# dohlee/rosettafold-pytorch

Measured on AMD Instinct MI355X. Metric: residues/sec forward (L=256, N=128), higher is better.
Workload: dtype bf16; 1 GPU; BASELINE.json configs[1]: bsz=4/GPU, n_seq=128, L=256, d_msa=384, d_pair=288, 8+5 blocks, 4 encoder layers, random-init weights; global_batch=4, parallelism=batch-sharded x1 (replicated weights), launch=one hipGraph replay per step (validation + input copy outside the graph)

## Files before the change

rosettafold-pytorch_amd/csrc/favor.hip:

```cpp
#include <type_traits>

#include "common.h"

#define FV_DH 64
#define FV_M 266
#define FV_MT 17
#define FV_MPAD 288
#define FV_CTX_LD 592
#define FV_DT 5
#define FV_DROWS 80

struct FavorAttnP {
  const h16_t* qkv;
  const h16_t* pc;
  h16_t* out;
  int64_t x_b, x_o, x_s;
  int64_t x_h;
  int64_t o_b, o_o, o_s;
  int q_off, k_off, v_off;
  int n_o, n_h, nitems;
  int nchunks;
  int dbg;
  float eps;
  float ctx_scale;
  int seq_len;
};

#ifdef RF_H16_IS_F16
#define FV_CS(x) ((x) * p.ctx_scale)
#else
#define FV_CS(x) (x)
#endif

typedef __attribute__((ext_vector_type(4))) short s16x4;

__device__ __forceinline__ int swz_off(int row, int chunk) { return row * 128 + ((chunk ^ (row & 7)) << 4); }

template <bool TAIL = false>
__device__ __forceinline__ void fv_load_tile(char* smem, int lds_off, const h16_t* g, int64_t stride, int nrows,
                                             int wave, int lane, int nvalid = 0) {
  const int ninstr = nrows * 8 / 64;
  for (int it = wave; it < ninstr; it += 4) {
    const int slot = it * 64 + lane;
    const int row = slot >> 3;
    const int clog = (slot & 7) ^ (row & 7);
    const int srow = TAIL ? (row < nvalid ? row : nvalid - 1) : row;
    rf_glds16(g + (int64_t)srow * stride + clog * 8, smem + lds_off + it * 1024);
  }
}

__device__ __forceinline__ float rbf(float x) { return h2f(f2h(x)); }

__device__ __forceinline__ float fv_mfma_done(float acc_reg) {
  asm volatile("s_nop 7\n\ts_nop 3" : "+v"(acc_reg));
  return acc_reg;
}

union Frag {
  h16x8 v;
  unsigned u[4];
  uint2 h[2];
};

template <int LS, bool SOFTMAX, bool TAIL>
__global__ __launch_bounds__(256, 1) void favor_attention_kernel(const FavorAttnP p) {
  constexpr int ST = LS / 64;
  constexpr int NSB = LS / 32;
  constexpr int PC_OFF = 0;
  constexpr int K_OFF = FV_MPAD * 128;
  constexpr int V_OFF = K_OFF + LS * 128;
  constexpr int CTX_OFF = V_OFF + LS * 128;
  constexpr int DIAG_OFF = CTX_OFF + FV_DROWS * FV_CTX_LD;
  constexpr int RED_OFF = DIAG_OFF + LS * 4;
  extern __shared__ __attribute__((aligned(16))) char smem[];
  const int tid = threadIdx.x, lane = tid & 63;
  const int wave = __builtin_amdgcn_readfirstlane(tid >> 6) & 3;
  const int fr = lane & 15, fq = lane >> 4;
  const int nm = wave == 0 ? 5 : 4;
  const int m0t = wave == 0 ? 0 : 5 + 4 * (wave - 1);
  const f32x4 epsv = {p.eps, p.eps, p.eps, p.eps};
  Frag ones;
#pragma unroll
  for (int k = 0; k < 4; ++k) ones.u[k] = fr == 0 ? RF_H16_ONE2 : 0u;

  fv_load_tile(smem, PC_OFF, p.pc, FV_DH, FV_MPAD, wave, lane);
  for (int i = tid; i < FV_DROWS * FV_CTX_LD / 4; i += 256) ((unsigned*)(smem + CTX_OFF))[i] = 0u;

  auto item_base = [&](int item, int64_t& xb, int64_t& ob) {
    const int h = item % p.n_h;
    const int t = item / p.n_h;
    const int o = t % p.n_o, b = t / p.n_o;
    xb = (int64_t)b * p.x_b + (int64_t)o * p.x_o + (int64_t)h * p.x_h;
    ob = (int64_t)b * p.o_b + (int64_t)o * p.o_o + h * FV_DH;
  };

  const int nch = p.nchunks;
  const int nv = TAIL ? p.seq_len : 0;
  int item = blockIdx.x;
  if (item < p.nitems) {
    int64_t xb, ob;
    item_base(item, xb, ob);
    fv_load_tile<TAIL>(smem, K_OFF, p.qkv + xb + p.k_off, p.x_s, LS, wave, lane, nv);
    fv_load_tile<TAIL>(smem, V_OFF, p.qkv + xb + p.v_off, p.x_s, LS, wave, lane, nv);
  }
  bool first = true;
  for (; item < p.nitems; item += gridDim.x) {
    int64_t xb, ob;
    item_base(item, xb, ob);
    if (first || TAIL)
      asm volatile("s_waitcnt vmcnt(0)" ::: "memory");
    else
      asm volatile("s_waitcnt vmcnt(%0)" ::"n"(ST * 4) : "memory");
    first = false;
    __syncthreads();
    h16x8 qf[ST][2];
    auto load_q = [&](int chunk) {
#pragma unroll
      for (int t = 0; t < ST; ++t) {
        int s = chunk * LS + (wave * ST + t) * 16 + fr;
        if (TAIL) s = s < nv ? s : nv - 1;
        const h16_t* qrow = p.qkv + xb + p.q_off + (int64_t)s * p.x_s;
#pragma unroll
        for (int kk = 0; kk < 2; ++kk) qf[t][kk] = *(const h16x8*)(qrow + (kk * 4 + fq) * 8);
      }
    };
    load_q(0);

    float gmax = 0.f;
    if constexpr (SOFTMAX) {
      for (int s = tid; s < LS; s += 256) {
        float a = 0.f;
#pragma unroll
        for (int c = 0; c < 8; ++c) {
          const h16x8 x = *(const h16x8*)(smem + K_OFF + s * 128 + c * 16);
#pragma unroll
          for (int e = 0; e < 8; ++e) {
            const float f = h2f((h16_t)x[e]);
            a = fmaf(f, f, a);
          }
        }
        ((float*)(smem + DIAG_OFF))[s] = a * (0.0625f * 1.4426950408889634f);
      }
    }

    h16x8 pf[5][2];
#pragma unroll
    for (int j = 0; j < 5; ++j)
#pragma unroll
      for (int kk = 0; kk < 2; ++kk)
        if (j < nm) pf[j][kk] = *(const h16x8*)(smem + PC_OFF + swz_off((m0t + j) * 16 + fr, kk * 4 + fq));

    if constexpr (SOFTMAX) {
      float mx = -INFINITY;
      const int nsb0 = TAIL ? (nv + 31) >> 5 : NSB;
      for (int u = 0; u < nsb0; ++u) {
        h16x8 kf[2][2];
#pragma unroll
        for (int t = 0; t < 2; ++t)
#pragma unroll
          for (int kk = 0; kk < 2; ++kk)
            kf[t][kk] = *(const h16x8*)(smem + K_OFF + swz_off((2 * u + t) * 16 + fr, kk * 4 + fq));
#pragma unroll
        for (int j = 0; j < 5; ++j) {
          if (j < nm) {
            const bool valid = (m0t + j) * 16 + fr < FV_M;
#pragma unroll
            for (int t = 0; t < 2; ++t) {
              f32x4 a = {0.f, 0.f, 0.f, 0.f};
              a = rf_mfma16(kf[t][0], pf[j][0], a, 0, 0, 0);
              a = rf_mfma16(kf[t][1], pf[j][1], a, 0, 0, 0);
              if (valid) mx = fmaxf(mx, fmaxf(fmaxf(a[0], a[1]), fmaxf(a[2], a[3])));
            }
          }
        }
      }
      mx = wave_max(mx);
      if (lane == 0) ((float*)(smem + RED_OFF))[wave] = mx;
      __syncthreads();
      const float* red = (const float*)(smem + RED_OFF);
      gmax = fmaxf(fmaxf(red[0], red[1]), fmaxf(red[2], red[3]));
    }

    f32x4 ctx[5][FV_DT];
#pragma unroll
    for (int j = 0; j < 5; ++j)
#pragma unroll
      for (int i = 0; i < FV_DT; ++i) ctx[j][i] = (f32x4){0.f, 0.f, 0.f, 0.f};
    for (int ck = 0; ck < nch; ++ck) {
    const int rem = TAIL ? nv - ck * LS : LS;
    if (ck > 0) {
      __syncthreads();
      fv_load_tile<TAIL>(smem, K_OFF, p.qkv + xb + p.k_off + (int64_t)ck * LS * p.x_s, p.x_s, LS, wave, lane, rem);
      fv_load_tile<TAIL>(smem, V_OFF, p.qkv + xb + p.v_off + (int64_t)ck * LS * p.x_s, p.x_s, LS, wave, lane, rem);
      asm volatile("s_waitcnt vmcnt(0)" ::: "memory");
      __syncthreads();
    }
    const int nsb = TAIL ? (rem < LS ? (rem + 31) >> 5 : NSB) : NSB;
    for (int u = 0; u < nsb; ++u) {
      h16x8 kf[2][2];
#pragma unroll
      for (int t = 0; t < 2; ++t)
#pragma unroll
        for (int kk = 0; kk < 2; ++kk)
          kf[t][kk] = *(const h16x8*)(smem + K_OFF + swz_off((2 * u + t) * 16 + fr, kk * 4 + fq));
      Frag vf[4];
      {
        const int p4 = fr & 3;
#pragma unroll
        for (int i = 0; i < 4; ++i) {
#pragma unroll
          for (int half = 0; half < 2; ++half) {
            const int row = u * 32 + half * 16 + 4 * fq + (fr >> 2);
            const int off = V_OFF + swz_off(row, i * 2 + (p4 >> 1)) + (p4 & 1) * 8;
            const s16x4 r = __builtin_amdgcn_ds_read_tr16_b64_v4i16((__attribute__((address_space(3))) s16x4*)(smem + off));
            vf[i].h[half] = __builtin_bit_cast(uint2, r);
          }
        }
      }
      f32x4 init[2] = {epsv, epsv};
      if constexpr (SOFTMAX) {
#pragma unroll
        for (int t = 0; t < 2; ++t) {
          const float4 d4 = *(const float4*)(smem + DIAG_OFF + ((2 * u + t) * 16 + 4 * fq) * 4);
          init[t] = (f32x4){-(d4.x + gmax), -(d4.y + gmax), -(d4.z + gmax), -(d4.w + gmax)};
        }
      }
#pragma unroll
      for (int j = 0; j < 5; ++j) {
        if (j < nm) {
          f32x4 a[2];
#pragma unroll
          for (int t = 0; t < 2; ++t) {
            a[t] = rf_mfma16(kf[t][0], pf[j][0], init[t], 0, 0, 0);
            a[t] = rf_mfma16(kf[t][1], pf[j][1], a[t], 0, 0, 0);
          }
          float f[2][4];
#pragma unroll
          for (int t = 0; t < 2; ++t)
#pragma unroll
            for (int r = 0; r < 4; ++r) {
              if constexpr (SOFTMAX)
                f[t][r] = __builtin_amdgcn_exp2f(a[t][r]) + p.eps;
              else
                f[t][r] = fmaxf(a[t][r], p.eps);
            }
          if ((m0t + j) == FV_MT - 1 && fr >= FV_M - 16 * (FV_MT - 1)) {
#pragma unroll
            for (int t = 0; t < 2; ++t)
#pragma unroll
              for (int r = 0; r < 4; ++r) f[t][r] = 0.f;
          }
          if constexpr (TAIL) {
            if ((u + 1) * 32 > rem) {
#pragma unroll
              for (int t = 0; t < 2; ++t)
#pragma unroll
                for (int r = 0; r < 4; ++r) f[t][r] = (2 * u + t) * 16 + 4 * fq + r < rem ? f[t][r] : 0.f;
            }
          }
          Frag kfr;
          kfr.u[0] = rf_pack2_h16(f[0][0], f[0][1]);
          kfr.u[1] = rf_pack2_h16(f[0][2], f[0][3]);
          kfr.u[2] = rf_pack2_h16(f[1][0], f[1][1]);
          kfr.u[3] = rf_pack2_h16(f[1][2], f[1][3]);
#pragma unroll
          for (int i = 0; i < 4; ++i)
            ctx[j][i] = rf_mfma16(kfr.v, vf[i].v, ctx[j][i], 0, 0, 0);
          ctx[j][4] = rf_mfma16(kfr.v, ones.v, ctx[j][4], 0, 0, 0);
        }
      }
    }
    }
#pragma unroll
    for (int j = 0; j < 5; ++j) {
      if (j < nm) {
#pragma unroll
        for (int i = 0; i < FV_DT; ++i) {
          uint2 w;
          w.x = rf_pack2_h16(FV_CS(ctx[j][i][0]), FV_CS(ctx[j][i][1]));
          w.y = rf_pack2_h16(FV_CS(ctx[j][i][2]), FV_CS(ctx[j][i][3]));
          *(uint2*)(smem + CTX_OFF + (i * 16 + fr) * FV_CTX_LD + ((m0t + j) * 16 + 4 * fq) * 2) = w;
        }
      }
    }
    __syncthreads();

    asm volatile("s_waitcnt vmcnt(0)" ::: "memory");
    {
      const int nxt = item + gridDim.x;
      if (nxt < p.nitems) {
        int64_t xb2, ob2;
        item_base(nxt, xb2, ob2);
        fv_load_tile<TAIL>(smem, K_OFF, p.qkv + xb2 + p.k_off, p.x_s, LS, wave, lane, nv);
        fv_load_tile<TAIL>(smem, V_OFF, p.qkv + xb2 + p.v_off, p.x_s, LS, wave, lane, nv);
      }
    }

    f32x4 qinit[ST];
#pragma unroll
    for (int t = 0; t < ST; ++t) qinit[t] = epsv;
    if constexpr (SOFTMAX) {
      float dq[ST], rmax[ST];
#pragma unroll
      for (int t = 0; t < ST; ++t) {
        float a = 0.f;
#pragma unroll
        for (int kk = 0; kk < 2; ++kk)
#pragma unroll
          for (int e = 0; e < 8; ++e) {
            const float f = h2f((h16_t)qf[t][kk][e]);
            a = fmaf(f, f, a);
          }
        a += __shfl_xor(a, 16, 64);
        a += __shfl_xor(a, 32, 64);
        dq[t] = a * (0.0625f * 1.4426950408889634f);
        rmax[t] = -INFINITY;
      }
      for (int j = 0; j < FV_MT; ++j) {
        h16x8 pfr[2];
#pragma unroll
        for (int kk = 0; kk < 2; ++kk) pfr[kk] = *(const h16x8*)(smem + PC_OFF + swz_off(j * 16 + fr, kk * 4 + fq));
#pragma unroll
        for (int t = 0; t < ST; ++t) {
          f32x4 a = {0.f, 0.f, 0.f, 0.f};
          a = rf_mfma16(pfr[0], qf[t][0], a, 0, 0, 0);
          a = rf_mfma16(pfr[1], qf[t][1], a, 0, 0, 0);
#pragma unroll
          for (int r = 0; r < 4; ++r)
            if (j * 16 + 4 * fq + r < FV_M) rmax[t] = fmaxf(rmax[t], a[r]);
        }
      }
#pragma unroll
      for (int t = 0; t < ST; ++t) {
        rmax[t] = fmaxf(rmax[t], __shfl_xor(rmax[t], 16, 64));
        rmax[t] = fmaxf(rmax[t], __shfl_xor(rmax[t], 32, 64));
        const float off = -(dq[t] + rmax[t]);
        qinit[t] = (f32x4){off, off, off, off};
      }
    }
    for (int qc = 0; qc < nch; ++qc) {
    if (TAIL && qc * LS + wave * ST * 16 >= nv) continue;
    if (qc > 0) load_q(qc);
    f32x4 num[FV_DT][ST];
#pragma unroll
    for (int t = 0; t < ST; ++t)
#pragma unroll
      for (int i = 0; i < FV_DT; ++i) num[i][t] = (f32x4){0.f, 0.f, 0.f, 0.f};
    auto mblock = [&](int u, auto last_tag) {
      constexpr bool LAST = decltype(last_tag)::value;
      float f[2][ST][4];
#pragma unroll
      for (int jj = 0; jj < 2; ++jj) {
        if (LAST && jj == 1) {
#pragma unroll
          for (int t = 0; t < ST; ++t)
#pragma unroll
            for (int r = 0; r < 4; ++r) f[jj][t][r] = 0.f;
        } else {
          const int j = 2 * u + jj;
          h16x8 pfr[2];
#pragma unroll
          for (int kk = 0; kk < 2; ++kk) pfr[kk] = *(const h16x8*)(smem + PC_OFF + swz_off(j * 16 + fr, kk * 4 + fq));
#pragma unroll
          for (int t = 0; t < ST; ++t) {
            f32x4 a = rf_mfma16(pfr[0], qf[t][0], qinit[t], 0, 0, 0);
            a = rf_mfma16(pfr[1], qf[t][1], a, 0, 0, 0);
#pragma unroll
            for (int r = 0; r < 4; ++r) {
              float x;
              if constexpr (SOFTMAX)
                x = __builtin_amdgcn_exp2f(a[r]) + p.eps;
              else
                x = fmaxf(a[r], p.eps);
              if (LAST && 4 * fq + r >= FV_M - 16 * (FV_MT - 1)) x = 0.f;
              f[jj][t][r] = x;
            }
          }
        }
      }
      Frag cf[FV_DT];
#pragma unroll
      for (int i = 0; i < FV_DT; ++i) {
        const char* base = smem + CTX_OFF + (i * 16 + fr) * FV_CTX_LD + (32 * u + 4 * fq) * 2;
        cf[i].h[0] = *(const uint2*)base;
        cf[i].h[1] = *(const uint2*)(base + 32);
      }
#pragma unroll
      for (int t = 0; t < ST; ++t) {
        Frag qfr;
        qfr.u[0] = rf_pack2_h16(f[0][t][0], f[0][t][1]);
        qfr.u[1] = rf_pack2_h16(f[0][t][2], f[0][t][3]);
        qfr.u[2] = rf_pack2_h16(f[1][t][0], f[1][t][1]);
        qfr.u[3] = rf_pack2_h16(f[1][t][2], f[1][t][3]);
#pragma unroll
        for (int i = 0; i < FV_DT; ++i)
          num[i][t] = rf_mfma16(cf[i].v, qfr.v, num[i][t], 0, 0, 0);
      }
    };
    for (int u = 0; u < (FV_MT - 1) / 2; ++u) mblock(u, std::false_type{});
    mblock((FV_MT - 1) / 2, std::true_type{});
#pragma unroll
    for (int t = 0; t < ST; ++t) {
      const float dn = __shfl(fv_mfma_done(num[4][t][0]), fr, 64);
      const float inv = 1.f / dn;
      const int s = qc * LS + (wave * ST + t) * 16 + fr;
      h16_t* orow = p.out + ob + (int64_t)s * p.o_s;
#pragma unroll
      for (int i = 0; i < 4; ++i) {
        uint2 w;
        w.x = rf_pack2_h16(num[i][t][0] * inv, num[i][t][1] * inv);
        w.y = rf_pack2_h16(num[i][t][2] * inv, num[i][t][3] * inv);
        if (!TAIL || s < nv) *(uint2*)(orow + i * 16 + 4 * fq) = w;
      }
    }
    }
  }
}

#pragma clang diagnostic ignored "-Winline-asm"
__device__ __forceinline__ void fv_glds_asm(const void* src, unsigned lds_addr) {
  asm volatile("s_mov_b32 m0, %0\n\ts_nop 0\n\tglobal_load_lds_dwordx4 %1, off" ::"s"(lds_addr), "v"(src) : "memory", "m0");
}

__device__ __forceinline__ void fv_lds_barrier() {
  asm volatile("s_waitcnt lgkmcnt(0)" ::: "memory");
  __builtin_amdgcn_s_barrier();
  asm volatile("" ::: "memory");
}

__device__ unsigned long long g_fv_cycles[8];
#define FV_STAMP(slot)                                                   \
  if (prof) {                                                            \
    const unsigned long long now = __builtin_readcyclecounter();         \
    acc_cyc[slot] += now - t_last;                                       \
    t_last = now;                                                        \
  }

template <int LS, bool SOFTMAX, bool TAIL>
__global__ __launch_bounds__(512, 1) void favor_attention_kernel8(const FavorAttnP p) {
  constexpr int NSB = LS / 32;
  constexpr int NJ = 3;
  constexpr int STB = LS >= 128 ? LS / 128 : 1;
  constexpr int NWB = LS / (16 * STB);
  constexpr int PC_OFF = 0;
  constexpr int K_OFF = FV_MPAD * 128;
  constexpr int V_OFF = K_OFF + LS * 128;
  constexpr int CTX_OFF = V_OFF + LS * 128;
  constexpr int DIAG_OFF = CTX_OFF + FV_DROWS * FV_CTX_LD;
  constexpr int RED_OFF = DIAG_OFF + LS * 4;
  extern __shared__ __attribute__((aligned(16))) char smem[];
  const int tid = threadIdx.x, lane = tid & 63;
  const int wave = __builtin_amdgcn_readfirstlane(tid >> 6) & 7;
  const int fr = lane & 15, fq = lane >> 4;
  const int nm = wave == 0 ? 3 : 2;
  const int m0t = wave == 0 ? 0 : 1 + 2 * wave;
  const f32x4 epsv = {p.eps, p.eps, p.eps, p.eps};
  Frag ones;
#pragma unroll
  for (int k = 0; k < 4; ++k) ones.u[k] = fr == 0 ? RF_H16_ONE2 : 0u;

  const unsigned lds_base = (unsigned)(uintptr_t)(__attribute__((address_space(3))) char*)smem;
  auto load_tile8 = [&](int lds_off, const h16_t* gp, int64_t stride, auto nrows_tag, int nvalid = 0) {
    constexpr int NI = decltype(nrows_tag)::value * 8 / 64;
    int ln = lane;
    asm volatile("" : "+v"(ln));
    const int dma_row = ln >> 3;
    const int dma_col = ((ln & 7) ^ dma_row) * 8;
    const h16_t* g0 = gp + (int64_t)dma_row * stride + dma_col;
#pragma unroll
    for (int k = 0; k < (NI + 7) / 8; ++k) {
      const int it = wave + 8 * k;
      if (NI % 8 == 0 || it < NI) {
        const unsigned dst = __builtin_amdgcn_readfirstlane(lds_base + lds_off + it * 1024);
        if (TAIL && nvalid > 0) {
          const int row = dma_row + 8 * it;
          fv_glds_asm(gp + (int64_t)(row < nvalid ? row : nvalid - 1) * stride + dma_col, dst);
        } else {
          fv_glds_asm(g0 + (int64_t)(8 * it) * stride, dst);
        }
      }
    }
  };
  constexpr std::integral_constant<int, LS> LS_TAG{};
  load_tile8(PC_OFF, p.pc, FV_DH, std::integral_constant<int, FV_MPAD>{});
  for (int i = tid; i < FV_DROWS * FV_CTX_LD / 4; i += 512) ((unsigned*)(smem + CTX_OFF))[i] = 0u;

  auto item_base = [&](int item, int64_t& xb, int64_t& ob) {
    const int h = item % p.n_h;
    const int t = item / p.n_h;
    const int o = t % p.n_o, b = t / p.n_o;
    xb = (int64_t)b * p.x_b + (int64_t)o * p.x_o + (int64_t)h * p.x_h;
    ob = (int64_t)b * p.o_b + (int64_t)o * p.o_o + h * FV_DH;
  };
  auto ctx_col = [](int tile, int q4) { return ((tile >> 1) * 32 + 8 * q4 + 4 * (tile & 1)) * 2; };
  const int nch = SOFTMAX ? 1 : p.nchunks;
  const int nv = TAIL ? p.seq_len : 0;
  int item = blockIdx.x;
  if (item < p.nitems) {
    int64_t xb, ob;
    item_base(item, xb, ob);
    load_tile8(K_OFF, p.qkv + xb + p.k_off, p.x_s, LS_TAG, nv);
    load_tile8(V_OFF, p.qkv + xb + p.v_off, p.x_s, LS_TAG, nv);
  }
  bool first = true;
  const bool prof = (RF_DBG(p.dbg) & 8) && wave == ((RF_DBG(p.dbg) >> 4) & 7);
  unsigned long long acc_cyc[7] = {0, 0, 0, 0, 0, 0, 0};
  unsigned long long t_last = prof ? __builtin_readcyclecounter() : 0;
  for (; item < p.nitems; item += gridDim.x) {
    int64_t xb, ob;
    item_base(item, xb, ob);
    asm volatile("" : "+v"(xb), "+v"(ob));
    if (prof) {
      t_last = __builtin_readcyclecounter();
      acc_cyc[6] += 1;
    }
    if (first || wave >= NWB || TAIL)
      asm volatile("s_waitcnt vmcnt(0)" ::: "memory");
    else
      asm volatile("s_waitcnt vmcnt(%0)" ::"n"(STB * 4) : "memory");
    first = false;
    fv_lds_barrier();
    FV_STAMP(0)
    h16x8 pf[NJ][2];
    {
      int frP = fr, fqP = fq;
      asm volatile("" : "+v"(frP), "+v"(fqP));
#pragma unroll
      for (int j = 0; j < NJ; ++j)
#pragma unroll
        for (int kk = 0; kk < 2; ++kk)
          pf[j][kk] = *(const h16x8*)(smem + PC_OFF + m0t * 2048 + swz_off(frP, kk * 4 + fqP) + (j < nm ? j : 0) * 2048);
    }
    h16x8 qf[STB][2];
    auto load_q = [&](int chunk) {
      int frq = fr, fqq = fq;
      asm volatile("" : "+v"(frq), "+v"(fqq));
      if (wave < NWB) {
#pragma unroll
        for (int t = 0; t < STB; ++t) {
          int s = chunk * LS + (wave * STB + t) * 16 + frq;
          if (TAIL) s = s < nv ? s : nv - 1;
          const h16_t* qrow = p.qkv + xb + p.q_off + (int64_t)s * p.x_s;
#pragma unroll
          for (int kk = 0; kk < 2; ++kk) qf[t][kk] = *(const h16x8*)(qrow + (kk * 4 + fqq) * 8);
        }
      }
    };
    load_q(0);

    float gmax = 0.f;
    if constexpr (SOFTMAX) {
      int frS = fr, fqS = fq;
      asm volatile("" : "+v"(frS), "+v"(fqS));
      for (int s = tid; s < LS; s += 512) {
        float a = 0.f;
#pragma unroll
        for (int c = 0; c < 8; ++c) {
          const h16x8 x = *(const h16x8*)(smem + K_OFF + s * 128 + c * 16);
#pragma unroll
          for (int e = 0; e < 8; ++e) {
            const float f = h2f((h16_t)x[e]);
            a = fmaf(f, f, a);
          }
        }
        ((float*)(smem + DIAG_OFF))[s] = a * (0.0625f * 1.4426950408889634f);
      }
      float mx = -INFINITY;
      const int nsb0 = TAIL ? (nv + 31) >> 5 : NSB;
      for (int u = 0; u < nsb0; ++u) {
        h16x8 kf[2][2];
#pragma unroll
        for (int t = 0; t < 2; ++t)
#pragma unroll
          for (int kk = 0; kk < 2; ++kk)
            kf[t][kk] = *(const h16x8*)(smem + K_OFF + swz_off((2 * u + t) * 16 + frS, kk * 4 + fqS));
#pragma unroll
        for (int j = 0; j < NJ; ++j) {
          if (j < nm) {
            const h16x8* pfj = pf[j];
            const bool valid = (m0t + j) != FV_MT - 1 || frS < FV_M - 16 * (FV_MT - 1);
#pragma unroll
            for (int t = 0; t < 2; ++t) {
              f32x4 a = {0.f, 0.f, 0.f, 0.f};
              a = rf_mfma16(kf[t][0], pfj[0], a, 0, 0, 0);
              a = rf_mfma16(kf[t][1], pfj[1], a, 0, 0, 0);
              if (valid) mx = fmaxf(mx, fmaxf(fmaxf(a[0], a[1]), fmaxf(a[2], a[3])));
            }
          }
        }
      }
      mx = wave_max(mx);
      if (lane == 0) ((float*)(smem + RED_OFF))[wave] = mx;
      fv_lds_barrier();
      const float* red = (const float*)(smem + RED_OFF);
      gmax = fmaxf(fmaxf(fmaxf(red[0], red[1]), fmaxf(red[2], red[3])), fmaxf(fmaxf(red[4], red[5]), fmaxf(red[6], red[7])));
    }

    f32x4 ctx[NJ][FV_DT];
#pragma unroll
    for (int j = 0; j < NJ; ++j)
#pragma unroll
      for (int i = 0; i < FV_DT; ++i) ctx[j][i] = (f32x4){0.f, 0.f, 0.f, 0.f};
    for (int ck = 0; ck < nch; ++ck) {
      const int rem = TAIL ? nv - ck * LS : LS;
      if (ck > 0) {
        __syncthreads();
        load_tile8(K_OFF, p.qkv + xb + p.k_off + (int64_t)ck * LS * p.x_s, p.x_s, LS_TAG, rem);
        load_tile8(V_OFF, p.qkv + xb + p.v_off + (int64_t)ck * LS * p.x_s, p.x_s, LS_TAG, rem);
        asm volatile("s_waitcnt vmcnt(0)" ::: "memory");
        __syncthreads();
      }
      const int nsb = TAIL ? (rem < LS ? (rem + 31) >> 5 : NSB) : NSB;
      h16x8 kf[2][2];
      Frag vf[4];
      auto load_sblock = [&](int u, h16x8 (&kfo)[2][2], Frag (&vfo)[4]) {
#pragma unroll
        for (int t = 0; t < 2; ++t)
#pragma unroll
          for (int kk = 0; kk < 2; ++kk)
            kfo[t][kk] = *(const h16x8*)(smem + K_OFF + swz_off((2 * u + t) * 16 + fr, kk * 4 + fq));
        const int p4 = fr & 3;
#pragma unroll
        for (int i = 0; i < 4; ++i) {
#pragma unroll
          for (int half = 0; half < 2; ++half) {
            const int row = u * 32 + half * 16 + 4 * fq + (fr >> 2);
            const int off = V_OFF + swz_off(row, i * 2 + (p4 >> 1)) + (p4 & 1) * 8;
            const s16x4 r = __builtin_amdgcn_ds_read_tr16_b64_v4i16((__attribute__((address_space(3))) s16x4*)(smem + off));
            vfo[i].h[half] = __builtin_bit_cast(uint2, r);
          }
        }
      };
      load_sblock(0, kf, vf);
      for (int u = 0; u < ((RF_DBG(p.dbg) & 1) ? 0 : nsb); ++u) {
        h16x8 kfn[2][2];
        Frag vfn[4];
        load_sblock(u + 1 < nsb ? u + 1 : u, kfn, vfn);
        f32x4 init[2] = {epsv, epsv};
        if constexpr (SOFTMAX) {
#pragma unroll
          for (int t = 0; t < 2; ++t) {
            const float4 d4 = *(const float4*)(smem + DIAG_OFF + ((2 * u + t) * 16 + 4 * fq) * 4);
            init[t] = (f32x4){-(d4.x + gmax), -(d4.y + gmax), -(d4.z + gmax), -(d4.w + gmax)};
          }
        }
#pragma unroll
        for (int j = 0; j < NJ; ++j) {
          if (j < nm) {
            const h16x8* pfj = pf[j];
            f32x4 a[2];
#pragma unroll
            for (int t = 0; t < 2; ++t) {
              a[t] = rf_mfma16(kf[t][0], pfj[0], init[t], 0, 0, 0);
              a[t] = rf_mfma16(kf[t][1], pfj[1], a[t], 0, 0, 0);
            }
            float f[2][4];
#pragma unroll
            for (int t = 0; t < 2; ++t)
#pragma unroll
              for (int r = 0; r < 4; ++r) {
                if constexpr (SOFTMAX)
                  f[t][r] = __builtin_amdgcn_exp2f(a[t][r]) + p.eps;
                else
                  f[t][r] = fmaxf(a[t][r], p.eps);
              }
            if ((m0t + j) == FV_MT - 1 && fr >= FV_M - 16 * (FV_MT - 1)) {
#pragma unroll
              for (int t = 0; t < 2; ++t)
#pragma unroll
                for (int r = 0; r < 4; ++r) f[t][r] = 0.f;
            }
            if constexpr (TAIL) {
              if ((u + 1) * 32 > rem) {
#pragma unroll
                for (int t = 0; t < 2; ++t)
#pragma unroll
                  for (int r = 0; r < 4; ++r) f[t][r] = (2 * u + t) * 16 + 4 * fq + r < rem ? f[t][r] : 0.f;
              }
            }
            Frag kfr;
            kfr.u[0] = rf_pack2_h16(f[0][0], f[0][1]);
            kfr.u[1] = rf_pack2_h16(f[0][2], f[0][3]);
            kfr.u[2] = rf_pack2_h16(f[1][0], f[1][1]);
            kfr.u[3] = rf_pack2_h16(f[1][2], f[1][3]);
#pragma unroll
            for (int i = 0; i < 4; ++i)
              ctx[j][i] = rf_mfma16(kfr.v, vf[i].v, ctx[j][i], 0, 0, 0);
            ctx[j][4] = rf_mfma16(kfr.v, ones.v, ctx[j][4], 0, 0, 0);
          }
        }
#pragma unroll
        for (int t = 0; t < 2; ++t)
#pragma unroll
          for (int kk = 0; kk < 2; ++kk) kf[t][kk] = kfn[t][kk];
#pragma unroll
        for (int i = 0; i < 4; ++i) vf[i] = vfn[i];
      }
    }
    FV_STAMP(1)
#pragma unroll
    for (int j = 0; j < NJ; ++j)
      if (j < nm) {
#pragma unroll
        for (int i = 0; i < FV_DT; ++i) {
          uint2 w;
          w.x = rf_pack2_h16(FV_CS(ctx[j][i][0]), FV_CS(ctx[j][i][1]));
          w.y = rf_pack2_h16(FV_CS(ctx[j][i][2]), FV_CS(ctx[j][i][3]));
          *(uint2*)(smem + CTX_OFF + (i * 16 + fr) * FV_CTX_LD + ctx_col(m0t + j, fq)) = w;
        }
      }
    fv_lds_barrier();
    FV_STAMP(2)
    asm volatile("s_waitcnt vmcnt(0)" ::: "memory");
#pragma unroll
    for (int t = 0; t < STB; ++t) {
      asm volatile("" : "+v"(qf[t][0]), "+v"(qf[t][1]));
    }
    {
      const int nxt = item + gridDim.x;
      if (nxt < p.nitems) {
        int64_t xb2, ob2;
        item_base(nxt, xb2, ob2);
        load_tile8(K_OFF, p.qkv + xb2 + p.k_off, p.x_s, LS_TAG, nv);
        load_tile8(V_OFF, p.qkv + xb2 + p.v_off, p.x_s, LS_TAG, nv);
      }
    }
    FV_STAMP(3)
    for (int qc = 0; qc < nch; ++qc) {
      if (qc > 0) {
        load_q(qc);
        asm volatile("s_waitcnt vmcnt(0)" ::: "memory");
#pragma unroll
        for (int t = 0; t < STB; ++t) {
          asm volatile("" : "+v"(qf[t][0]), "+v"(qf[t][1]));
        }
      }
      if (wave < NWB && (!TAIL || qc * LS + wave * STB * 16 < nv)) {
        f32x4 qinit[STB];
#pragma unroll
        for (int t = 0; t < STB; ++t) qinit[t] = epsv;
        if constexpr (SOFTMAX) {
          float dq[STB], rmax[STB];
#pragma unroll
          for (int t = 0; t < STB; ++t) {
            float a = 0.f;
#pragma unroll
            for (int kk = 0; kk < 2; ++kk)
#pragma unroll
              for (int e = 0; e < 8; ++e) {
                const float f = h2f((h16_t)qf[t][kk][e]);
                a = fmaf(f, f, a);
              }
            a += __shfl_xor(a, 16, 64);
            a += __shfl_xor(a, 32, 64);
            dq[t] = a * (0.0625f * 1.4426950408889634f);
            rmax[t] = -INFINITY;
          }
          for (int j = 0; j < FV_MT; ++j) {
            h16x8 pfr[2];
#pragma unroll
            for (int kk = 0; kk < 2; ++kk) pfr[kk] = *(const h16x8*)(smem + PC_OFF + swz_off(j * 16 + fr, kk * 4 + fq));
#pragma unroll
            for (int t = 0; t < STB; ++t) {
              f32x4 a = {0.f, 0.f, 0.f, 0.f};
              a = rf_mfma16(pfr[0], qf[t][0], a, 0, 0, 0);
              a = rf_mfma16(pfr[1], qf[t][1], a, 0, 0, 0);
#pragma unroll
              for (int r = 0; r < 4; ++r)
                if (j * 16 + 4 * fq + r < FV_M) rmax[t] = fmaxf(rmax[t], a[r]);
            }
          }
#pragma unroll
          for (int t = 0; t < STB; ++t) {
            rmax[t] = fmaxf(rmax[t], __shfl_xor(rmax[t], 16, 64));
            rmax[t] = fmaxf(rmax[t], __shfl_xor(rmax[t], 32, 64));
            const float off = -(dq[t] + rmax[t]);
            qinit[t] = (f32x4){off, off, off, off};
          }
        }
        f32x4 num[FV_DT][STB];
#pragma unroll
        for (int t = 0; t < STB; ++t)
#pragma unroll
          for (int i = 0; i < FV_DT; ++i) num[i][t] = (f32x4){0.f, 0.f, 0.f, 0.f};
        auto mblock = [&](int u, auto last_tag) {
          constexpr bool LAST = decltype(last_tag)::value;
          float f[2][STB][4];
#pragma unroll
          for (int jj = 0; jj < 2; ++jj) {
            if (LAST && jj == 1) {
#pragma unroll
              for (int t = 0; t < STB; ++t)
#pragma unroll
                for (int r = 0; r < 4; ++r) f[jj][t][r] = 0.f;
            } else {
              const int j = 2 * u + jj;
              h16x8 pfr[2];
#pragma unroll
              for (int kk = 0; kk < 2; ++kk) pfr[kk] = *(const h16x8*)(smem + PC_OFF + swz_off(j * 16 + fr, kk * 4 + fq));
#pragma unroll
              for (int t = 0; t < STB; ++t) {
                f32x4 a = rf_mfma16(pfr[0], qf[t][0], qinit[t], 0, 0, 0);
                a = rf_mfma16(pfr[1], qf[t][1], a, 0, 0, 0);
#pragma unroll
                for (int r = 0; r < 4; ++r) {
                  float x;
                  if constexpr (SOFTMAX)
                    x = __builtin_amdgcn_exp2f(a[r]) + p.eps;
                  else
                    x = fmaxf(a[r], p.eps);
                  if (LAST && 4 * fq + r >= FV_M - 16 * (FV_MT - 1)) x = 0.f;
                  f[jj][t][r] = x;
                }
              }
            }
          }
          Frag cf[FV_DT];
#pragma unroll
          for (int i = 0; i < FV_DT; ++i)
            cf[i].v = *(const h16x8*)(smem + CTX_OFF + (i * 16 + fr) * FV_CTX_LD + (32 * u + 8 * fq) * 2);
#pragma unroll
          for (int t = 0; t < STB; ++t) {
            Frag qfr;
            qfr.u[0] = rf_pack2_h16(f[0][t][0], f[0][t][1]);
            qfr.u[1] = rf_pack2_h16(f[0][t][2], f[0][t][3]);
            qfr.u[2] = rf_pack2_h16(f[1][t][0], f[1][t][1]);
            qfr.u[3] = rf_pack2_h16(f[1][t][2], f[1][t][3]);
#pragma unroll
            for (int i = 0; i < FV_DT; ++i)
              num[i][t] = rf_mfma16(cf[i].v, qfr.v, num[i][t], 0, 0, 0);
          }
        };
        for (int u = 0; u < ((RF_DBG(p.dbg) & 2) ? 0 : (FV_MT - 1) / 2); ++u) mblock(u, std::false_type{});
        mblock((FV_MT - 1) / 2, std::true_type{});
        FV_STAMP(4)
#pragma unroll
        for (int t = 0; t < STB; ++t) {
          const float dn = __shfl(fv_mfma_done(num[4][t][0]), fr, 64);
          const float inv = 1.f / dn;
          const int s = qc * LS + (wave * STB + t) * 16 + fr;
          h16_t* orow = p.out + ob + (int64_t)s * p.o_s;
#pragma unroll
          for (int i = 0; i < 4; ++i) {
            uint2 w;
            w.x = rf_pack2_h16(num[i][t][0] * inv, num[i][t][1] * inv);
            w.y = rf_pack2_h16(num[i][t][2] * inv, num[i][t][3] * inv);
            if (!TAIL || s < nv) *(uint2*)(orow + i * 16 + 4 * fq) = w;
          }
        }
      }
    }
    FV_STAMP(5)
  }
  if (prof && lane == 0) {
#pragma unroll
    for (int i = 0; i < 7; ++i) atomicAdd(&g_fv_cycles[i], acc_cyc[i]);
  }
}

extern "C" int rf_favor_phase_cycles(unsigned long long* out7, int reset) {
  unsigned long long z[8] = {0, 0, 0, 0, 0, 0, 0, 0};
  if (out7 && hipMemcpyFromSymbol(out7, HIP_SYMBOL(g_fv_cycles), 7 * sizeof(unsigned long long)) != hipSuccess) return 1000 + (int)hipGetLastError();
  if (reset && hipMemcpyToSymbol(HIP_SYMBOL(g_fv_cycles), z, sizeof(z)) != hipSuccess) return 1000 + (int)hipGetLastError();
  return 0;
}

template <int LS, bool SM, bool TAIL>
static int launch_favor(const FavorAttnP& p, hipStream_t s) {
  const size_t lds = (size_t)FV_MPAD * 128 + 2 * (size_t)LS * 128 + (size_t)FV_DROWS * FV_CTX_LD + LS * 4 + 64;
  const int ncu = rf_num_cus() > 0 ? rf_num_cus() : 256;
  const int grid = p.nitems < ncu ? p.nitems : ncu;
  static const bool force4 = getenv("RF_FAVOR4") != nullptr;
  constexpr bool only4 = SM && LS > 128;
  if (only4 || force4) {
    auto k = favor_attention_kernel<LS, SM, TAIL>;
    if (const int e = rf_enable_big_lds<favor_attention_kernel<LS, SM, TAIL>>()) return e;
    hipLaunchKernelGGL(k, dim3(grid), dim3(256), lds, s, p);
  } else if constexpr (!only4) {
    auto k = favor_attention_kernel8<LS, SM, TAIL>;
    if (const int e = rf_enable_big_lds<favor_attention_kernel8<LS, SM, TAIL>>()) return e;
    hipLaunchKernelGGL(k, dim3(grid), dim3(512), lds, s, p);
  }
  return rf_launch_status();
}

extern "C" int rf_favor_attention(const void* qkv, const void* pc, void* out, const int64_t x_strides[4],
                                  const int64_t o_strides[3], int q_off, int k_off, int v_off, int n_b, int n_o,
                                  int n_h, int seq_len, int dim_head, int n_features, int softmax_kernel, float eps,
                                  void* stream) {
  if (dim_head != FV_DH || n_features != FV_M) return RF_EINVAL;
  if (seq_len < 1) return RF_EINVAL;
  int nchunks = 1, ls = seq_len <= 64 ? 64 : seq_len <= 128 ? 128 : 256;
  if (seq_len > 256) {
    if (softmax_kernel) return RF_EINVAL;
    nchunks = (seq_len + 255) / 256;
  }
  const bool tail = seq_len != nchunks * ls;
  if (((uintptr_t)qkv % 16) || ((uintptr_t)pc % 16) || ((uintptr_t)out % 8)) return RF_EALIGN;
  for (int i = 0; i < 3; ++i)
    if (x_strides[i] % 8 || o_strides[i] % 4) return RF_EALIGN;
  if (x_strides[3] % 8) return RF_EALIGN;
  if (q_off % 8 || k_off % 8 || v_off % 8) return RF_EALIGN;
  FavorAttnP p;
  p.qkv = (const h16_t*)qkv;
  p.pc = (const h16_t*)pc;
  p.out = (h16_t*)out;
  p.x_b = x_strides[0]; p.x_o = x_strides[1]; p.x_s = x_strides[2]; p.x_h = x_strides[3];
  p.o_b = o_strides[0]; p.o_o = o_strides[1]; p.o_s = o_strides[2];
  p.q_off = q_off; p.k_off = k_off; p.v_off = v_off;
  p.n_o = n_o; p.n_h = n_h;
  p.nitems = n_b * n_o * n_h;
  p.eps = eps;
  p.nchunks = nchunks;
  p.seq_len = seq_len;
  p.ctx_scale = 1.0f;
#ifdef RF_H16_IS_F16
  for (int n = 1; n < seq_len; n <<= 1) p.ctx_scale *= 0.5f;
#endif
  static int dbg = 0;
  static const int dbg_rc = rf_dbg_env("RF_FAVOR_DBG", &dbg);
  if (dbg_rc) return dbg_rc;
  p.dbg = dbg;
  hipStream_t s = (hipStream_t)stream;
#define FV_LAUNCH(LS_) \
  (tail ? (softmax_kernel ? launch_favor<LS_, true, true>(p, s) : launch_favor<LS_, false, true>(p, s)) \
        : (softmax_kernel ? launch_favor<LS_, true, false>(p, s) : launch_favor<LS_, false, false>(p, s)))
  if (ls == 256) return FV_LAUNCH(256);
  if (ls == 128) return FV_LAUNCH(128);
  return FV_LAUNCH(64);
#undef FV_LAUNCH
}
```

Measured before the change: 3211 residues/s.

## Split FAVOR K/V prefetch into halves to overlap refill with context accumulation

Adds a HALF variant of the 512-thread FAVOR attention kernel, used for aligned 256-row ReLU inputs. It walks the K/V context accumulation in two halves and starts DMA for the next item's first half of K/V tiles as soon as the current first half is consumed. The second half is issued after the context barrier. The aim is to hide more global-to-LDS load latency behind MFMA work than a single refill after the context pass does. The cost is an extra barrier per item and more intricate vmcnt accounting, including inline-asm Q loads so the wait counts stay exact.

```diff
diff --git a/rosettafold-pytorch_amd/csrc/favor.hip b/rosettafold-pytorch_amd/csrc/favor.hip
--- a/rosettafold-pytorch_amd/csrc/favor.hip
+++ b/rosettafold-pytorch_amd/csrc/favor.hip
@@ -436,8 +436,10 @@
     t_last = now;                                                        \
   }
 
-template <int LS, bool SOFTMAX, bool TAIL>
+template <int LS, bool SOFTMAX, bool TAIL, bool HALF = false>
 __global__ __launch_bounds__(512, 1) void favor_attention_kernel8(const FavorAttnP p) {
+  static_assert(!HALF || (LS == 256 && !SOFTMAX && !TAIL), "the half-tile refill covers the aligned 256-row ReLU instantiation");
+  constexpr int NDMA = LS / 32;
   constexpr int NSB = LS / 32;
   constexpr int NJ = 3;
   constexpr int STB = LS >= 128 ? LS / 128 : 1;
@@ -460,15 +462,18 @@
   for (int k = 0; k < 4; ++k) ones.u[k] = fr == 0 ? RF_H16_ONE2 : 0u;
 
   const unsigned lds_base = (unsigned)(uintptr_t)(__attribute__((address_space(3))) char*)smem;
-  auto load_tile8 = [&](int lds_off, const h16_t* gp, int64_t stride, auto nrows_tag, int nvalid = 0) {
+  auto load_tile8_part = [&](int lds_off, const h16_t* gp, int64_t stride, auto nrows_tag, int nvalid, auto part_tag) {
     constexpr int NI = decltype(nrows_tag)::value * 8 / 64;
+    constexpr int PART = decltype(part_tag)::value;
+    constexpr int KN = (NI + 7) / 8;
+    static_assert(PART == 0 || NI % 16 == 0, "halves: an even number of instructions per wave");
     int ln = lane;
     asm volatile("" : "+v"(ln));
     const int dma_row = ln >> 3;
     const int dma_col = ((ln & 7) ^ dma_row) * 8;
     const h16_t* g0 = gp + (int64_t)dma_row * stride + dma_col;
 #pragma unroll
-    for (int k = 0; k < (NI + 7) / 8; ++k) {
+    for (int k = (PART == 2 ? KN / 2 : 0); k < (PART == 1 ? KN / 2 : KN); ++k) {
       const int it = wave + 8 * k;
       if (NI % 8 == 0 || it < NI) {
         const unsigned dst = __builtin_amdgcn_readfirstlane(lds_base + lds_off + it * 1024);
@@ -481,6 +486,9 @@
       }
     }
   };
+  auto load_tile8 = [&](int lds_off, const h16_t* gp, int64_t stride, auto nrows_tag, int nvalid = 0) {
+    load_tile8_part(lds_off, gp, stride, nrows_tag, nvalid, std::integral_constant<int, 0>{});
+  };
   constexpr std::integral_constant<int, LS> LS_TAG{};
   load_tile8(PC_OFF, p.pc, FV_DH, std::integral_constant<int, FV_MPAD>{});
   for (int i = tid; i < FV_DROWS * FV_CTX_LD / 4; i += 512) ((unsigned*)(smem + CTX_OFF))[i] = 0u;
@@ -493,7 +501,7 @@
     ob = (int64_t)b * p.o_b + (int64_t)o * p.o_o + h * FV_DH;
   };
   auto ctx_col = [](int tile, int q4) { return ((tile >> 1) * 32 + 8 * q4 + 4 * (tile & 1)) * 2; };
-  const int nch = SOFTMAX ? 1 : p.nchunks;
+  const int nch = (SOFTMAX || HALF) ? 1 : p.nchunks;
   const int nv = TAIL ? p.seq_len : 0;
   int item = blockIdx.x;
   if (item < p.nitems) {
@@ -503,6 +511,15 @@
     load_tile8(V_OFF, p.qkv + xb + p.v_off, p.x_s, LS_TAG, nv);
   }
   bool first = true;
+  auto prefetch_next = [&](int item, auto part_tag) {
+    const int nxt = item + gridDim.x;
+    if (nxt < p.nitems) {
+      int64_t xb2, ob2;
+      item_base(nxt, xb2, ob2);
+      load_tile8_part(K_OFF, p.qkv + xb2 + p.k_off, p.x_s, LS_TAG, 0, part_tag);
+      load_tile8_part(V_OFF, p.qkv + xb2 + p.v_off, p.x_s, LS_TAG, 0, part_tag);
+    }
+  };
   const bool prof = (RF_DBG(p.dbg) & 8) && wave == ((RF_DBG(p.dbg) >> 4) & 7);
   unsigned long long acc_cyc[7] = {0, 0, 0, 0, 0, 0, 0};
   unsigned long long t_last = prof ? __builtin_readcyclecounter() : 0;
@@ -516,6 +533,8 @@
     }
     if (first || wave >= NWB || TAIL)
       asm volatile("s_waitcnt vmcnt(0)" ::: "memory");
+    else if constexpr (HALF)
+      asm volatile("s_waitcnt vmcnt(%0)" ::"n"(NDMA / 2 + STB * 4) : "memory");
     else
       asm volatile("s_waitcnt vmcnt(%0)" ::"n"(STB * 4) : "memory");
     first = false;
@@ -542,7 +561,12 @@
           if (TAIL) s = s < nv ? s : nv - 1;
           const h16_t* qrow = p.qkv + xb + p.q_off + (int64_t)s * p.x_s;
 #pragma unroll
-          for (int kk = 0; kk < 2; ++kk) qf[t][kk] = *(const h16x8*)(qrow + (kk * 4 + fqq) * 8);
+          for (int kk = 0; kk < 2; ++kk) {
+            if constexpr (HALF)
+              asm volatile("global_load_dwordx4 %0, %1, off" : "=&v"(qf[t][kk]) : "v"(qrow + (kk * 4 + fqq) * 8) : "memory");
+            else
+              qf[t][kk] = *(const h16x8*)(qrow + (kk * 4 + fqq) * 8);
+          }
         }
       }
     };
@@ -631,11 +655,26 @@
           }
         }
       };
-      load_sblock(0, kf, vf);
-      for (int u = 0; u < ((RF_DBG(p.dbg) & 1) ? 0 : nsb); ++u) {
+      for (int hf = 0; hf < (HALF ? 2 : 1); ++hf) {
+      const int u0 = HALF ? hf * (NSB / 2) : 0, u1 = HALF ? u0 + NSB / 2 : nsb;
+      if constexpr (HALF) {
+        if (hf == 1) {
+          FV_STAMP(1)
+          asm volatile("s_waitcnt vmcnt(0)" ::: "memory");
+#pragma unroll
+          for (int t = 0; t < STB; ++t) {
+            asm volatile("" : "+v"(qf[t][0]), "+v"(qf[t][1]));
+          }
+          fv_lds_barrier();
+          FV_STAMP(0)
+          prefetch_next(item, std::integral_constant<int, 1>{});
+        }
+      }
+      load_sblock(u0, kf, vf);
+      for (int u = u0; u < ((RF_DBG(p.dbg) & 1) ? u0 : u1); ++u) {
         h16x8 kfn[2][2];
         Frag vfn[4];
-        load_sblock(u + 1 < nsb ? u + 1 : u, kfn, vfn);
+        load_sblock(u + 1 < u1 ? u + 1 : u, kfn, vfn);
         f32x4 init[2] = {epsv, epsv};
         if constexpr (SOFTMAX) {
 #pragma unroll
@@ -696,6 +735,7 @@
 #pragma unroll
         for (int i = 0; i < 4; ++i) vf[i] = vfn[i];
       }
+      }
     }
     FV_STAMP(1)
 #pragma unroll
@@ -711,12 +751,14 @@
       }
     fv_lds_barrier();
     FV_STAMP(2)
-    asm volatile("s_waitcnt vmcnt(0)" ::: "memory");
-#pragma unroll
-    for (int t = 0; t < STB; ++t) {
-      asm volatile("" : "+v"(qf[t][0]), "+v"(qf[t][1]));
-    }
-    {
+    if constexpr (HALF) {
+      prefetch_next(item, std::integral_constant<int, 2>{});
+    } else {
+      asm volatile("s_waitcnt vmcnt(0)" ::: "memory");
+#pragma unroll
+      for (int t = 0; t < STB; ++t) {
+        asm volatile("" : "+v"(qf[t][0]), "+v"(qf[t][1]));
+      }
       const int nxt = item + gridDim.x;
       if (nxt < p.nitems) {
         int64_t xb2, ob2;
@@ -877,9 +919,18 @@
     if (const int e = rf_enable_big_lds<favor_attention_kernel<LS, SM, TAIL>>()) return e;
     hipLaunchKernelGGL(k, dim3(grid), dim3(256), lds, s, p);
   } else if constexpr (!only4) {
-    auto k = favor_attention_kernel8<LS, SM, TAIL>;
-    if (const int e = rf_enable_big_lds<favor_attention_kernel8<LS, SM, TAIL>>()) return e;
-    hipLaunchKernelGGL(k, dim3(grid), dim3(512), lds, s, p);
+    constexpr bool half = LS == 256 && !SM && !TAIL;
+    if (half && p.nchunks == 1) {
+      if constexpr (half) {
+        auto k = favor_attention_kernel8<LS, SM, false, true>;
+        if (const int e = rf_enable_big_lds<favor_attention_kernel8<LS, SM, false, true>>()) return e;
+        hipLaunchKernelGGL(k, dim3(grid), dim3(512), lds, s, p);
+      }
+    } else {
+      auto k = favor_attention_kernel8<LS, SM, TAIL>;
+      if (const int e = rf_enable_big_lds<favor_attention_kernel8<LS, SM, TAIL>>()) return e;
+      hipLaunchKernelGGL(k, dim3(grid), dim3(512), lds, s, p);
+    }
   }
   return rf_launch_status();
 }
```

Result: no change. 3194 residues/s (-0.5%).
